# humansensinglab/AGenDA

Measured on AMD Instinct MI355X. Metric: 512x512 images/sec + DAAM heatmaps, 50 DDIM steps, SD-1.5, higher is better.
Workload: dtype bf16

## Files before the change

agenda_amd/csrc/attention.hip:

```cpp
#include "kernels.h"
#include <type_traits>

#ifdef AGD_EXPERIMENTS
int g_attn_qb = 1;
extern "C" __attribute__((visibility("default"))) void agd_set_attn_qb(int v) { g_attn_qb = v; }
#else
constexpr int g_attn_qb = 1;
#endif

template <int D> struct AttnCfg {
  static constexpr int KSTEPS = (D + 15) / 16;
  static constexpr int DBLK = (D + 31) / 32;
  static constexpr int KCH = KSTEPS * 2;
  static constexpr int KPITCH = ((KCH | 1)) * 16;
  static constexpr int VPITCH = ((DBLK | 1)) * 64;
  static constexpr int CH = D / 8;
  static constexpr bool ONES = (DBLK * 32 > D);
  static constexpr bool QPAD = (KSTEPS * 16 > D);
};

#define DEFER_THR 8.0f

template <int D, int KB, int QB, int RECORD, int AMASK = 0, int EXTRA = 0>
#if defined(AGD_EXPERIMENTS) && defined(EXP_ATTN_LB)
#define ATTN_LB(def) ((!RECORD && !AMASK) ? EXP_ATTN_LB : (def))
#else
#define ATTN_LB(def) (def)
#endif
__global__ __launch_bounds__(256, ATTN_LB((AMASK ? 1 : (QB == 1 && D <= 64 && !RECORD) ? 3 : (QB == 1 && D <= 80) ? 2 : 1))) void attn_kernel(const AttnP p) {
  using C = AttnCfg<D>;
  constexpr int KEYS = KB * 32;
  constexpr int KSTEPS = C::KSTEPS, DBLK = C::DBLK, KPITCH = C::KPITCH, VPITCH = C::VPITCH, CH = C::CH;
  constexpr bool ONES = C::ONES && !RECORD;
  constexpr bool QPAD = C::QPAD && !RECORD;
  constexpr bool CNEG = !QPAD && !RECORD;
  constexpr int NCHUNK = KEYS * CH;
  constexpr int LD_IT = (NCHUNK + 255) / 256;
  constexpr int STAGE = KEYS * (KPITCH + VPITCH);
  constexpr int NSTAGE = (RECORD == 1) ? 1 : 2;
  extern __shared__ __attribute__((aligned(16))) char smem[];

  const int tid = threadIdx.x, lane = tid & 63, wid = tid >> 6;
  const int c = lane & 31, hh = lane >> 5;
  const int HPB = (RECORD == 2) ? p.H / p.rec_hpb : p.H;
  const int nqt = p.nqt, nbh = p.B * HPB;
  int bh, qt;
  {
    const int id = blockIdx.x, x = id & 7, j = id >> 3;
    const int per = (nbh + 7) >> 3;
    const int lb = j / nqt;
    qt = j - lb * nqt;
    bh = x * per + lb;
  }
  if (bh >= nbh) return;
  const int hgrp = bh % HPB;
  int head = (RECORD == 2) ? hgrp * p.rec_hpb : hgrp;
  const int hend = (RECORD == 2) ? head + p.rec_hpb : head + 1;
  const int b = bh / HPB;
  const int q0 = qt * (128 * QB) + wid * (32 * QB);
  const bf16_t* kp = p.k + b * p.sk + head * D;
  const bf16_t* vp = p.v + b * p.sv + head * D;

// ... 115 lines not shown
#pragma unroll
      for (int j = 0; j < 16; ++j) oacc[qb][i][j] = 0.f;
  float m_run[QB], l_run[QB];
  f32x16 negm[CNEG ? QB : 1];
#pragma unroll
  for (int qb = 0; qb < QB; ++qb) {
    m_run[qb] = RECORD ? -INFINITY : 0.f; l_run[qb] = 0.f;
    if constexpr (CNEG) {
#pragma unroll
      for (int j = 0; j < 16; ++j) negm[qb][j] = 0.f;
    }
  }
  const float sc = qscale;
  f32x16 pacc[RECORD == 2 ? KB : 1];
  const bool recb = RECORD == 2 && p.record_mode == 3 && b >= p.rec_b0;
  if constexpr (RECORD == 2) {
#pragma unroll
    for (int kb = 0; kb < KB; ++kb)
#pragma unroll
      for (int j = 0; j < 16; ++j) pacc[kb][j] = 0.f;
  }

  const int ntiles_main = RECORD ? 1 : (p.Nk + KEYS - 1) / KEYS;
  const int ntiles = ntiles_main + (EXTRA ? 1 : 0);
  const bool ragged = (p.Nk % KEYS) != 0 || p.causal || AMASK;
  gload(0);
  lstore(0);
  __syncthreads();

  const int gi = lane & 15;
  const int tr_row = (gi >> 2) + 4 * hh;
  const int tr_col = ((lane >> 4) & 1) * 16 + (gi & 3) * 4;

  auto tile_body = [&](int t, auto mask_tag) {
    constexpr bool MASK = decltype(mask_tag)::value;
    const int cur = (RECORD == 1) ? 0 : (RECORD == 2) ? ((t - (hend - p.rec_hpb)) & 1) : (t & 1);
    const char* sK = smem + cur * STAGE;
    const char* sV = sK + KEYS * KPITCH;
    if constexpr (RECORD == 2) { if (t + 1 < hend) { gload_head(t + 1); prefetch_q(t + 1); } }
    else if constexpr (EXTRA) { if (t + 1 < ntiles_main) gload(t + 1); else if (t + 1 == ntiles_main) gload_extra(); }
    else if (t + 1 < ntiles) gload(t + 1);
    f32x16 sacc[QB][KB];
#pragma unroll
    for (int kb = 0; kb < KB; ++kb) {
#pragma unroll
      for (int s = 0; s < KSTEPS; ++s) {
        const bf16x8 a = *(const bf16x8*)(sK + (kb * 32 + c) * KPITCH + (2 * s + hh) * 16);
#pragma unroll
        for (int qb = 0; qb < QB; ++qb) {
          if (s == 0) { const f32x16 z = {0.f, 0.f, 0.f, 0.f, 0.f, 0.f, 0.f, 0.f, 0.f, 0.f, 0.f, 0.f, 0.f, 0.f, 0.f, 0.f};
                        sacc[qb][kb] = __builtin_amdgcn_mfma_f32_32x32x16_bf16(a, qf[qb][s], CNEG ? negm[qb] : z, 0, 0, 0); }
          else sacc[qb][kb] = __builtin_amdgcn_mfma_f32_32x32x16_bf16(a, qf[qb][s], sacc[qb][kb], 0, 0, 0);
        }
      }
    }
    if constexpr (MASK) {
#pragma unroll
      for (int qb = 0; qb < QB; ++qb)
#pragma unroll
        for (int kb = 0; kb < KB; ++kb)
#pragma unroll
          for (int i = 0; i < 16; ++i) {
            const int key = (RECORD || (EXTRA && t == ntiles_main) ? 0 : t * KEYS) + kb * 32 + (i & 3) + 8 * (i >> 2) + 4 * hh;
            if (key >= ((EXTRA && t == ntiles_main) ? p.Nk2 : p.Nk) || (p.causal && key > q0 + qb * 32 + c)) sacc[qb][kb][i] = -INFINITY;
            else if constexpr (AMASK) {
              const float a = p.mask[(long long)b * p.Nk + key];
              sacc[qb][kb][i] += RECORD ? a / p.scale : a * 1.44269504088896340736f;
            }
          }
    }
#pragma unroll
    for (int qb = 0; qb < QB; ++qb) {
      float mx = sacc[qb][0][0];
#pragma unroll
      for (int kb = 0; kb < KB; ++kb)
#pragma unroll
        for (int i = 0; i < 16; ++i) mx = fmaxf(mx, sacc[qb][kb][i]);
      if constexpr (RECORD) {
        mx = xhalf_max(mx) * sc;
        m_run[qb] = mx;
        if constexpr (RECORD == 2) l_run[qb] = 0.f;
        const float nm = -mx;
        float rs = 0.f;
#pragma unroll
        for (int kb = 0; kb < KB; ++kb)
#pragma unroll
          for (int i = 0; i < 16; ++i) {
            const float pv = __builtin_amdgcn_exp2f(fmaf(sacc[qb][kb][i], sc, nm));
            sacc[qb][kb][i] = pv;
            rs += pv;
          }
        l_run[qb] += rs;
      } else {
        if (t == 0 || !__all(mx <= DEFER_THR)) {
          const float mxf = xhalf_max(mx);
          float delta = (t == 0) ? mxf : fmaxf(mxf, 0.f);
          if (!(delta > -INFINITY)) delta = 0.f;
          if constexpr (QPAD) {
            const float mb = (float)(__bf16)(m_run[qb] + delta);
            delta = mb - m_run[qb];
            constexpr int pc = D - 16 * (KSTEPS - 1);
            if (hh == pc / 8) qf[qb][KSTEPS - 1][pc % 8] = (__bf16)(-mb);
          }
          const float alpha = __builtin_amdgcn_exp2f(-delta);
          m_run[qb] += delta;
          l_run[qb] *= alpha;
#pragma unroll
          for (int db = 0; db < DBLK; ++db)
#pragma unroll
            for (int j = 0; j < 16; ++j) oacc[qb][db][j] *= alpha;
#pragma unroll
          for (int kb = 0; kb < KB; ++kb)
#pragma unroll
            for (int i = 0; i < 16; ++i) sacc[qb][kb][i] -= delta;
          if constexpr (CNEG) {
            const float nm = -m_run[qb];
#pragma unroll
            for (int j = 0; j < 16; ++j) negm[qb][j] = nm;
          }
        }
        if constexpr (CNEG) asm volatile("" : "+v"(negm[qb]));
        if constexpr (ONES) {
#pragma unroll
          for (int kb = 0; kb < KB; ++kb)
#pragma unroll
            for (int i = 0; i < 16; ++i) sacc[qb][kb][i] = __builtin_amdgcn_exp2f(sacc[qb][kb][i]);
        } else {
// ... 44 lines not shown
              __builtin_amdgcn_raw_buffer_store_b32(__builtin_bit_cast(unsigned, old[i] + sacc[0][kb][i] * inv), rsrc, off, 0, 0);
            }
          }
        }
      }
    }

#pragma unroll
    for (int kb = 0; kb < KB; ++kb)
#pragma unroll
      for (int s = 0; s < 2; ++s) {
        bf16x8 pf[QB];
#pragma unroll
        for (int qb = 0; qb < QB; ++qb)
#pragma unroll
          for (int j = 0; j < 8; ++j) pf[qb][j] = (__bf16)sacc[qb][kb][8 * s + j];
        const char* vb = sV + (kb * 32 + 16 * s + tr_row) * VPITCH + tr_col * 2;
#pragma unroll
        for (int db = 0; db < DBLK; ++db) {
          const s16x4 lo = __builtin_amdgcn_ds_read_tr16_b64_v4i16((__attribute__((address_space(3))) s16x4*)(vb + db * 64));
          const s16x4 hi = __builtin_amdgcn_ds_read_tr16_b64_v4i16((__attribute__((address_space(3))) s16x4*)(vb + 8 * VPITCH + db * 64));
          const u32x2 lo2 = __builtin_bit_cast(u32x2, lo), hi2 = __builtin_bit_cast(u32x2, hi);
          const u32x4 a4 = u32x4{lo2[0], lo2[1], hi2[0], hi2[1]};
#pragma unroll
          for (int qb = 0; qb < QB; ++qb)
            oacc[qb][db] = __builtin_amdgcn_mfma_f32_32x32x16_bf16(__builtin_bit_cast(bf16x8, a4), pf[qb], oacc[qb][db], 0, 0, 0);
        }
      }
    if ((RECORD == 2) ? (t + 1 < hend) : (t + 1 < ntiles)) {
      lstore(cur ^ 1);
      __syncthreads();
    }
  };
  auto store_o = [&]() {
#pragma unroll
    for (int qb = 0; qb < QB; ++qb) {
      float lt;
      if constexpr (ONES) {
        constexpr int ld = D % 32;
        const float lv = oacc[qb][D / 32][4 * (ld / 8)];
        lt = __shfl(lv, c);
      } else {
        lt = xhalf_sum(l_run[qb]);
      }
      const float inv = 1.0f / lt;
      const int qrow = q0 + qb * 32 + c;
      if (qrow < p.Nq) {
        bf16_t* op = p.o + b * p.so + (long long)qrow * p.ldo + head * D;
#pragma unroll
        for (int db = 0; db < DBLK; ++db)
#pragma unroll
          for (int g = 0; g < 4; ++g) {
            const int d0 = db * 32 + 8 * g + 4 * hh;
            if (d0 < D) {
              u32x2 pk;
              pk[0] = pack_bf2(oacc[qb][db][4 * g + 0] * inv, oacc[qb][db][4 * g + 1] * inv);
              pk[1] = pack_bf2(oacc[qb][db][4 * g + 2] * inv, oacc[qb][db][4 * g + 3] * inv);
              *(u32x2*)(op + d0) = pk;
            }
          }
      }
    }
  };
  {
    using T_ = std::integral_constant<bool, true>; using F_ = std::integral_constant<bool, false>;
    if constexpr (RECORD == 2) {
      const int h0 = head;
      for (; head < hend; ++head) {
        if (head > h0) {
#pragma unroll
          for (int s = 0; s < KSTEPS; ++s) qf[0][s] = __builtin_bit_cast(bf16x8, qnext[s]);
#pragma unroll
          for (int db = 0; db < DBLK; ++db)
#pragma unroll
            for (int j = 0; j < 16; ++j) oacc[0][db][j] = 0.f;
        }
        tile_body(head, T_{});
        store_o();
      }
      if (recb && (q0 + c) < p.Nq) {
        float* base = p.rec + (long long)(b - p.rec_b0) * p.rec_img_stride + hgrp * p.rec_head_stride;
        const unsigned nbytes = (unsigned)p.rec_T * (unsigned)p.Nq * 4u;
        const auto rsrc = __builtin_amdgcn_make_buffer_rsrc(base, 0, nbytes, 0x00020000);
        const unsigned rowb = (unsigned)p.Nq * 4u;
        const unsigned voff0 = (unsigned)(q0 + c) * 4u + (unsigned)(4 * hh) * rowb;
        float old[KB][16];
#pragma unroll
        for (int kb = 0; kb < KB; ++kb)
#pragma unroll
          for (int i = 0; i < 16; ++i)
            old[kb][i] = __builtin_bit_cast(float, __builtin_amdgcn_raw_buffer_load_b32(rsrc, voff0 + (unsigned)(kb * 32 + (i & 3) + 8 * (i >> 2)) * rowb, 0, 0));
#pragma unroll
        for (int kb = 0; kb < KB; ++kb)
#pragma unroll
          for (int i = 0; i < 16; ++i)
            __builtin_amdgcn_raw_buffer_store_b32(__builtin_bit_cast(unsigned, old[kb][i] + pacc[kb][i]), rsrc,
                                                  voff0 + (unsigned)(kb * 32 + (i & 3) + 8 * (i >> 2)) * rowb, 0, 0);
      }
      return;
    } else if constexpr (RECORD) {
      tile_body(0, T_{});
    } else if constexpr (EXTRA) {
      for (int t = 0; t < ntiles_main - 1; ++t) tile_body(t, F_{});
      if (ragged) tile_body(ntiles_main - 1, T_{}); else tile_body(ntiles_main - 1, F_{});
      tile_body(ntiles_main, T_{});
    } else {
      if (p.causal || AMASK) { for (int t = 0; t < ntiles - 1; ++t) tile_body(t, T_{}); }
      else { for (int t = 0; t < ntiles - 1; ++t) tile_body(t, F_{}); }
      if (ragged) tile_body(ntiles - 1, T_{}); else tile_body(ntiles - 1, F_{});
    }
  }
  store_o();
}


template <int D, int KB, int QB, int RECORD, int AMASK = 0, int EXTRA = 0>
static int launch_attn_t(const AttnP& p, hipStream_t st) {
  using C = AttnCfg<D>;
  constexpr int lds = (RECORD == 1 ? 1 : 2) * KB * 32 * (C::KPITCH + C::VPITCH);
  AttnP pp = p;
  pp.nqt = (p.Nq + 128 * QB - 1) / (128 * QB);
  const int per = (p.B * (RECORD == 2 ? p.H / p.rec_hpb : p.H) + 7) / 8;
  dim3 grid(8 * per * pp.nqt);
  auto kfn = attn_kernel<D, KB, QB, RECORD, AMASK, EXTRA>;
  if (lds > 65536) {
    static std::atomic<bool> attr[AGD_MAX_DEVICES] = {};
    int dev = 0; HIP_CHECK_RET(hipGetDevice(&dev));
    if (dev < 0 || dev >= AGD_MAX_DEVICES) { agd_set_error("attention: device ordinal %d out of range", dev); return -1; }
    if (!attr[dev]) { HIP_CHECK_RET(hipFuncSetAttribute((const void*)kfn, hipFuncAttributeMaxDynamicSharedMemorySize, lds)); attr[dev] = true; }
  }
  hipLaunchKernelGGL(kfn, grid, dim3(256), lds, st, pp);
  HIP_CHECK_RET(hipGetLastError());
  return 0;
}

template <int D>
static int launch_attn_d(const AttnP& p, hipStream_t st) {
  if (p.k2) {
    if (p.record_mode != 0 || p.mask || p.causal) { agd_set_error("attention: a second K/V source takes no recording, mask or causal order"); return -1; }
    if (!p.v2 || p.Nk2 < 1 || p.Nk2 > 64 || ((p.ldk2 | p.ldv2) & 7)) { agd_set_error("attention: second K/V source of %d keys (1 .. 64, pitches multiples of 8)", p.Nk2); return -1; }
    return launch_attn_t<D, 2, 1, 0, 0, 1>(p, st);
  }
  if (p.record_mode != 0) {
    if (p.Nk > 96) { agd_set_error("attention: recording needs Nk <= 96 (got %d)", p.Nk); return -1; }
    if (p.record_mode == 3) {
      if (p.mask) { agd_set_error("attention: head-summed recording does not take an attention mask"); return -1; }
      if (p.rec_hpb < 1 || p.H % p.rec_hpb) { agd_set_error("attention: rec_hpb %d does not divide %d heads", p.rec_hpb, p.H); return -1; }
      return launch_attn_t<D, 3, 1, 2>(p, st);
    }
    return p.mask ? launch_attn_t<D, 3, 1, 1, 1>(p, st) : launch_attn_t<D, 3, 1, 1>(p, st);
  }
  if (p.mask) {
    if (p.causal) { agd_set_error("attention: additive mask + causal unsupported"); return -1; }
    return (p.Nk <= 96 && p.Nk > 64) ? launch_attn_t<D, 3, 1, 0, 1>(p, st) : launch_attn_t<D, 2, 1, 0, 1>(p, st);
  }
  if (p.Nk <= 96 && p.Nk > 64) return launch_attn_t<D, 3, 1, 0>(p, st);
  if constexpr (D <= 80) { if (p.Nq >= 1024 && g_attn_qb == 2) return launch_attn_t<D, 2, 2, 0>(p, st); }
#if defined(AGD_EXPERIMENTS) && defined(EXP_ATTN_KB)
  if (p.Nk >= 1024) return launch_attn_t<D, EXP_ATTN_KB, 1, 0>(p, st);
#endif
  return launch_attn_t<D, 2, 1, 0>(p, st);
}

int launch_attention(const AttnP& p, hipStream_t st) {
  if ((p.ldq | p.ldk | p.ldv | p.ldo) & 3) { agd_set_error("attention: row pitches must be multiples of 4 elements"); return -1; }
  if ((p.ldq | p.ldk | p.ldv) & 7) { agd_set_error("attention: q/k/v pitches must be multiples of 8 elements"); return -1; }
  switch (p.D) {
    case 32: return launch_attn_d<32>(p, st);
    case 40: return launch_attn_d<40>(p, st);
    case 64: return launch_attn_d<64>(p, st);
    case 80: return launch_attn_d<80>(p, st);
    case 128: return launch_attn_d<128>(p, st);
    case 160: return launch_attn_d<160>(p, st);
    default: agd_set_error("attention: unsupported head dim %d", p.D); return -1;
  }
}
```

agenda_amd/csrc/kernels.h:

```cpp
#pragma once
#include "common.h"

#define AGD_MAX_DEVICES 16
struct SplitKWs { float* p = nullptr; size_t cap = 0; };

struct IgemmP {
  const bf16_t* sc0 = nullptr; const bf16_t* sc1 = nullptr; int sc_C0 = 0, sc_C1 = 0;
  int ups4 = 0;
  const bf16_t* src0; const bf16_t* src1;
  int C0, C1;
  int Hin, Win, Hout, Wout;
  int ksize, stride, pad, up;
  const bf16_t* W;
  const float* bias; int bias_mode;
  const float* rowadd; int rowadd_ld;
  const bf16_t* residual; int ldr;
  void* out; int out_f32; int ldo;
  int M, N, K;
  float alpha;
  int geglu;
  int act;
  int batch;
  long long sA0, sA1, sW, sO, sR;
  const bf16_t* zero_page;
// ... 6 lines not shown
  int* cfg_out;
  int w_per_image;
  int wmajor;
  int warm;
  int halo;
  int p8;
  const float* gn_gamma; const float* gn_beta; bf16_t* gn_y; int gn_groups; float gn_eps; int gn_silu; int gn_keep_out; int* gn_fused;
  int kg2;
  int smap;
  int wreg, wreg_mmin, wreg_mmax;
  const bf16_t* Wfrag; int wfrag_ni;
  int xb_m, xb_n;
  int xcd_block;
  int pc;
  int stagger;
  int dbg;
};
int launch_igemm(const IgemmP& p, hipStream_t st);
int igemm_query(const IgemmP& p, int* cfg3);

struct AttnP {
  const bf16_t* q; const bf16_t* k; const bf16_t* v; bf16_t* o;
  int ldq, ldk, ldv, ldo;
  long long sq, sk, sv, so;
  int B, H, D, Nq, Nk;
  float scale;
  int record_mode; int rec_b0;
  float* rec; long long rec_img_stride; long long rec_head_stride;
  int rec_T;
  int rec_hpb;
  int nqt;
  int causal;
  const float* mask;
  const bf16_t* k2; const bf16_t* v2; int ldk2, ldv2; long long sk2, sv2; int Nk2;
};
int launch_attention(const AttnP& p, hipStream_t st);

struct FFusedP {
  const bf16_t* h; bf16_t* out;
  const bf16_t* w1f;
  const float* cs1; const float* b1;
  const bf16_t* w2f;
  const float* b2;
  int M; float ln_eps;
  const bf16_t* wpf; const float* bp; const bf16_t* xres; bf16_t* pout; float* colstat;
  int xres_rows;
  int premul;
};
int launch_ff_fused(const FFusedP& p, int C, hipStream_t st);
struct AttnChainP {
  const bf16_t* h; bf16_t* out;
  const float* gamma; const float* beta; float ln_eps;
  const bf16_t* wqf;
  const bf16_t* wof; const float* bo;
  const bf16_t* kv; int ldkv; long long skv;
  int M, HW, T; float scale;
  int record; float* rec; long long rec_img_stride, rec_head_stride; int rec_T, rec_b0, rec_hpb;
  float* rowstat_out;
  const bf16_t* o1; const bf16_t* wo1f; const float* bo1;
  int rows32;
  int src_rows;
};
int launch_attn_chain(const AttnChainP& p, int C, int heads, hipStream_t st);
struct QkvChainP {
  const bf16_t* x;
  const bf16_t* wbf; long long wb_stride; const float* rowadd;
// ... 154 lines not shown
```

agenda_amd/csrc/model.hip:

```cpp
#include "../../include/agenda_hip.h"
#include "kernels.h"

#include <algorithm>
#include <cmath>
#include <cstdarg>
#include <cstdio>
#include <cstring>
#include <functional>
#include <string>
#include <unordered_map>
#include <vector>

static thread_local char g_err[2048] = "";
#define AGD_API extern "C" __attribute__((visibility("default")))
extern "C" void agd_set_error(const char* fmt, ...) {
  va_list ap; va_start(ap, fmt); vsnprintf(g_err, sizeof(g_err), fmt, ap); va_end(ap);
}
#define CK(expr) do { if ((expr) != 0) return -1; } while (0)
#define FAIL(...) do { agd_set_error(__VA_ARGS__); return -1; } while (0)

struct WMat { bf16_t* w = nullptr; int N = 0, Cin = 0, Cpad = 0, taps = 0;
              int sc_cols = 0;
              bf16_t* wfrag = nullptr; int wfrag_ni = 0; };
struct Act { bf16_t* p = nullptr; int B = 0, H = 0, W = 0, C = 0; float* cpart = nullptr; int cpart_bm = 0;
// ... 38 lines not shown
  int acc_heads = 0;
  DBuf wqTb, wkvTb, woTb; WMat wqT, wkvT, woT;
  bf16_t* pm_wqT = nullptr; float* pm_wqb = nullptr; bool pm_ready = false;
  DBuf pm_kppb, pm_vppb, pm_csb; bf16_t* pm_kpp = nullptr; bf16_t* pm_vpp = nullptr; float* pm_kcs = nullptr; float* pm_kbs = nullptr;
};

struct Fuser {
  std::string pre; int C = 0, heads = 0;
  WMat wqkv, wkv; float ta = 0.f, td = 0.f; float* bo_s = nullptr; float* b2_s = nullptr;
  DBuf gkvb;
};

struct IpaLayer {
  std::string pre; int C = 0, heads = 0, cols = 0;
  DBuf wk, wv, kppb, vppb, csbsb;
};

enum : int {
  TBF_FF            = 1 << 0,
  TBF_ATTN2         = 1 << 1,
  TBF_ATTN1_OUT     = 1 << 2,
  TBF_FF_PROJ       = 1 << 3,
  TBF_QKV           = 1 << 4,
  TBF_ATTN2_640     = 1 << 5,
  TBF_LAZY_DUP      = 1 << 6,
  TBF_QKV_GN        = 1 << 7,
  TBF_QKV_640       = 1 << 8,
  TBF_FF_PREMUL     = 1 << 9,
  TBF_ATTN2_ROWS32  = 1 << 10,
  TBF_QKV_ROWS64    = 1 << 11,
  TBF_QKV_SCHED2    = 1 << 12,
  TBF_DEFAULT       = 0x1fff & ~TBF_QKV_640,
};

struct ProfEv { int cls; double flops, bytes; hipEvent_t a, b; };

struct EvalCond {
  float cn_scale = 0.f;
  bool grounded = false;
  float ad_scale = 0.f;
  bool ipa = false;
};

struct agd_ctx {
  int device = 0; agd_config cfg{}; std::string err;
  std::unordered_map<std::string, WMat> W;
  std::unordered_map<std::string, float*> V;
  std::unordered_map<std::string, int> Vn;
  std::vector<void*> owned;
  Arena arena; bf16_t* zero_page = nullptr;
  float* stage = nullptr; size_t stage_bytes = 0;
  bool finalized = false;
  WMat tproj_all; float* tproj_bias = nullptr; float* tproj_out = nullptr; int tproj_total = 0;
  const float* tproj_cur = nullptr;
  int tproj_cur_ld = 0;
  float* tsteps_buf = nullptr; int tsteps_cap = 0;
  std::unordered_map<std::string, int> tproj_off;
  float* temb_buf = nullptr;
  float* t_dev = nullptr;
  std::vector<XLayer> xl; std::unordered_map<std::string, int> xl_idx;
  DBuf ctxb; bf16_t* ctx_bf16 = nullptr; int ctx_B2 = 0, ctx_T = 0;
  int rec_mode = 0, rec_is_train = 0, rec_T_cfg = 0, rec_T = 0, rec_B = 0, rec_L = 0, rec_Lh = 0, rec_Lw = 0;
  DBuf hook_sumb, hook_scratchb, hook_headsb, hook_storeb;
  struct HookRec { size_t off; int Bp, T, N; };
  std::vector<HookRec> hook_recs; size_t hook_store_used = 0;
  DBuf bwd_wsb;
  float* hook_sum = nullptr; float* hook_scratch = nullptr; int hook_count = 0, hook_Bp = 0, hook_T = 0;
  int rec_base = 0, rec_call = 0;
  int pano_B = 0, pano_Lh = 0, pano_Lw = 0, pano_stride = 0;
  DBuf pano_ctxb;
  DBuf pano_viewb, pano_hmb;
  DBuf latb, epsb, vae_imgb, plmsb, dpmb;
  bf16_t* lat_bf16 = nullptr; float* eps_nhwc = nullptr;
  SplitKWs splitk;
  int opt_cfg_share = 1;
  int opt_ln_fold = 1;
  int opt_gn_fused = 1;
  int opt_warm = 3;
  int opt_gn_proj_fold = 1;
  int opt_p8 = 1;
  int opt_halo = 1;
  int opt_tb_fuse = TBF_DEFAULT;
  int opt_ups4 = 7;
  int opt_ffproj = 1;
  int opt_sc_fuse = 3;
  int opt_wreg = 3;
  int opt_kg2 = 1;
  int opt_side = 0;
  hipStream_t side = nullptr; hipEvent_t ev_fork = nullptr, ev_join = nullptr;
  int opt_smap = 1;
  int opt_reduce_gn = 1;
  int opt_xcd_block = 1;
  int opt_pc = 49;
  agd_vision_config vis{}; bool vis_on = false; float* vis_concepts = nullptr;
  agd_vision_config ienc{}; int ienc_state = 0;
  int opt_xpre = 1;
  int opt_touch = 3;
  unsigned* touch_sink = nullptr;
  agd_controlnet_config cnc{}; bool cn_on = false;
  WMat cn_tproj_all; float* cn_tproj_bias = nullptr; float* cn_tproj_out = nullptr; int cn_tproj_total = 0;
  int cn_nres = 0; float* cn_zb = nullptr; float* cn_zbs = nullptr; int cn_zb_total = 0; std::vector<int> cn_zb_off; float cn_zscale = NAN;
  DBuf cn_embb; int cn_emb_B2 = 0, cn_emb_Lh = 0, cn_emb_Lw = 0, cn_emb_rep = 0;
  std::vector<float> cn_sched;
  int ip_mode = 0, ip_B = 0, ip_Lh = 0, ip_Lw = 0, ip_Cm = 0, ip_Cc = 0;
  DBuf ip_maskb, ip_condb, ip_noiseb;
  std::vector<float> ip_sched;
  bool i2_on = false; int i2_B = 0, i2_Lh = 0, i2_Lw = 0; float i2_scale = 1.f;
  int i2_prep_B = 0, i2_prep_Lh = 0, i2_prep_Lw = 0;
  DBuf i2_latb;
  std::vector<std::string> lora_keys; std::vector<LoraMergeD> lora_d; int lora_tiles = 0;
  DBuf lora_descb; bf16_t* lora_scratch = nullptr; size_t lora_scratch_n = 0;
  float lora_scale = 0.f; bool lora_dirty = false;
// ... 253 lines not shown
    c->arena.release(mk);
    return 0;
  }
  if (side_out) {
    if (hipStreamWaitEvent(st, c->ev_join, 0) != hipSuccess) FAIL("side stream wait");
    res = side_out;
  } else if (has_sc) {
    GETW(ws, pre + "conv_shortcut.weight"); GETV(bs, pre + "conv_shortcut.bias");
    GemmOpt os; os.bias = bs;
    CK(run_conv(c, st, x0.p, x0.C, x1 ? x1->p : nullptr, C1, B, H, Wd, *ws, 1, h.p, os, c->zero_page));
    res = h.p;
  } else if (x1 || x0.C != Cout) {
    FAIL("resnet %s: channel change %d->%d without conv_shortcut", pre.c_str(), Cin, Cout);
  }
  GETW(w2, pre + "conv2.weight"); GETV(cb2, pre + "conv2.bias");
  GemmOpt o2; o2.bias = cb2; o2.residual = res; o2.out_act = &out;
  int gn2_done = 0;
  if (out_normed) {
    o2.gn_gamma = next->gamma; o2.gn_beta = next->beta; o2.gn_y = out_normed; o2.gn_groups = groups; o2.gn_eps = next->eps; o2.gn_silu = next->silu;
    o2.gn_keep_out = 1; o2.gn_fused = &gn2_done;
  }
  CK(run_conv(c, st, n2.p, Cout, nullptr, 0, B, H, Wd, *w2, 3, out.p, o2, c->zero_page));
  if (gn2_done) { out.normed = out_normed; out.normed_gamma = next->gamma; }
  c->arena.release(mk);
  return 0;
}

static int run_attention(agd_ctx* c, hipStream_t st, int cls, AttnP& a) {
  const double fl = 4.0 * a.B * a.H * (double)a.Nq * a.Nk * a.D;
  double by = 2.0 * a.B * a.H * (double)a.D * (2.0 * a.Nq + 2.0 * a.Nk);
  if (a.record_mode == 1) by += 8.0 * (a.B - a.rec_b0) * a.H * (double)a.rec_T * a.Nq;
  else if (a.record_mode == 2 || a.record_mode == 3) by += 8.0 * (a.B - a.rec_b0) * (double)a.rec_T * a.Nq;
  ProfScope ps(c, st, cls, fl, by);
  return launch_attention(a, st);
}

static inline bool daam_records(const agd_ctx* c, const XLayer& xl, int B2, int qh, int qw) {
  return c->rec_mode == 1 && !xl.mid && xl.acc && c->rec_Lh / qh != 8 && qh == xl.acc_h && qw == xl.acc_w && B2 / 2 == rec_images(c);
}

static int cross_attention(agd_ctx* c, hipStream_t st, XLayer& xl, const bf16_t* q, int B2, int N, int qh, int qw, bf16_t* out, bool record,
                           const float* mask = nullptr) {
  const int C = xl.C, D = C / xl.heads, T = c->ctx_T;
  if (xl.cn) record = false;
  AttnP a{}; a.q = q; a.k = xl.kv; a.v = xl.kv + C; a.o = out;
  a.ldq = C; a.ldk = 2 * C; a.ldv = 2 * C; a.ldo = C;
  a.sq = (long long)N * C; a.sk = (long long)T * 2 * C; a.sv = a.sk; a.so = a.sq;
  a.B = B2; a.H = xl.heads; a.D = D; a.Nq = N; a.Nk = T; a.scale = 1.0f / sqrtf((float)D);
  a.record_mode = 0; a.mask = mask;
  const int side = qh;
  bool hook_call = false;
  if (record && daam_records(c, xl, B2, qh, qw)) {
    a.rec_b0 = B2 / 2; a.rec_T = c->rec_T;
    a.rec_head_stride = (long long)c->rec_T * N; a.rec_img_stride = a.rec_head_stride * xl.acc_heads;
    a.rec = xl.acc + (size_t)c->rec_base * a.rec_img_stride;
    if (xl.acc_heads < xl.heads) {
      if (mask) FAIL("attention_mask together with daam recording at latent resolution is not supported");
      a.record_mode = 3; a.rec_hpb = xl.heads / xl.acc_heads;
    } else a.record_mode = 1;
  } else if (record && c->rec_mode == 2 && c->hook_scratch) {
    const int b0 = c->rec_is_train ? 0 : B2 / 2;
    if (B2 - b0 == c->hook_Bp) {
      if (qh != qw) FAIL("the hook.py recorder takes square maps only (h = w = sqrt(N)); this call's map is %d x %d", qh, qw);
      if (T != c->hook_T || side > c->rec_L) FAIL("hook recorder was reset for %d tokens / latent side %d but this call has %d tokens / side %d: call clear() (agd_record_reset) after changing the context", c->hook_T, c->rec_L, T, side);
      const size_t nh = (size_t)c->hook_Bp * xl.heads * T * N;
      CK(c->hook_headsb.ensure(nh * 4));
// ... 1819 lines not shown
    const float* f; CK(guidance_factor(c, st, eps, batch, Cl, HW, guidance, &f));
    return launch_cfg_dpm(eps, c->cfg.out_channels, latents, prev, store, batch, Cl, HW, guidance, coeffs + (size_t)5 * i, f, st);
  }));
  return 0;
}
AGD_API int agd_denoise_dpm(agd_ctx* c, float* latents, int batch, int L, int n_evals, const float* timesteps, const float* coeffs,
                            float guidance, void* stream) {
  return agd_denoise_dpm_hw(c, latents, batch, L, L, n_evals, timesteps, coeffs, guidance, stream);
}

AGD_API int agd_vae_decode_hw(agd_ctx* c, const float* latents, int batch, int Lh, int Lw, unsigned char* out_u8, float* out_f32, void* stream) {
  API_CK(c, need_final(c));
  if (Lh < 1 || Lw < 1) { agd_set_error("vae_decode: latent size %d x %d", Lh, Lw); return fail_ctx(c); }
  hipStream_t st = S(stream);
  API_CK(c, ensure_lat(c, batch, Lh, Lw));
  const int sh = c->cfg.vae_n_levels - 1;
  const long long npix = (long long)batch * (Lh << sh) * (Lw << sh);
  { ProfScope ps(c, st, PC_ELEM, 0);
    API_CK(c, launch_prep_latents(latents, c->lat_bf16, batch, c->cfg.vae_latent_channels, Lh * Lw, 64, 1, 1.0f / c->cfg.vae_scaling_factor, st)); }
  API_CK(c, c->vae_imgb.ensure((size_t)npix * 4 * 4));
  float* img = c->vae_imgb.as<float>();
  int rc = vae_walk(c, st, c->lat_bf16, batch, Lh, Lw, img);
  if (rc == 0 && out_u8) { ProfScope ps(c, st, PC_ELEM, 0); rc = launch_image_u8(img, 4, out_u8, npix, c->cfg.vae_out_channels, st); }
  if (rc == 0 && out_f32) {
    rc = launch_nchw_from_nhwc_f32(img, 4, out_f32, (int)npix, c->cfg.vae_out_channels, 1, st);
  }
  return rc ? fail_ctx(c) : 0;
}
AGD_API int agd_vae_decode(agd_ctx* c, const float* latents, int batch, int L, unsigned char* out_u8, float* out_f32, void* stream) {
  return agd_vae_decode_hw(c, latents, batch, L, L, out_u8, out_f32, stream);
}

AGD_API int agd_set_option(agd_ctx* c, const char* name, int value) {
  if (!c || !name) { agd_set_error("set_option: null argument"); return fail_ctx(c); }
  if (!strcmp(name, "cfg_shared_prefix")) { c->opt_cfg_share = value != 0; return 0; }
  if (!strcmp(name, "ln_fold")) { c->opt_ln_fold = value; return 0; }
  if (!strcmp(name, "gn_fused_stats")) { c->opt_gn_fused = value != 0; return 0; }
  if (!strcmp(name, "weight_touch")) { c->opt_touch = value < 0 ? 0 : value; return 0; }
  if (!strcmp(name, "weight_warm")) { c->opt_warm = value; return 0; }
  if (!strcmp(name, "conv_halo")) { c->opt_halo = value != 0; return 0; }
  if (!strcmp(name, "gn_proj_fold")) { c->opt_gn_proj_fold = value < 0 ? 0 : value; return 0; }
  if (!strcmp(name, "tblock_fuse")) { c->opt_tb_fuse = value < 0 ? 0 : value; return 0; }
  if (!strcmp(name, "reduce_gn")) { c->opt_reduce_gn = value != 0; return 0; }
  if (!strcmp(name, "xcd_block")) { c->opt_xcd_block = value != 0; return 0; }
  if (!strcmp(name, "igemm_pc")) { c->opt_pc = value < 0 ? 0 : value; return 0; }
  if (!strcmp(name, "attn2_premul")) { c->opt_xpre = value < 0 ? 0 : value; return 0; }
  if (!strcmp(name, "conv_smap")) { c->opt_smap = value != 0; return 0; }
  if (!strcmp(name, "side_stream")) { c->opt_side = value < 0 ? 0 : value; return 0; }
  if (!strcmp(name, "igemm_kgroups")) { c->opt_kg2 = value != 0; return 0; }
  if (!strcmp(name, "upsample_phases")) { c->opt_ups4 = value & 15; return 0; }
  if (!strcmp(name, "ff_proj_fuse")) { c->opt_ffproj = value != 0; return 0; }
  if (!strcmp(name, "shortcut_fuse")) { c->opt_sc_fuse = value & 3; return 0; }
  if (!strcmp(name, "wreg_mask")) { c->opt_wreg = value & 3; return 0; }
  if (!strcmp(name, "igemm8p")) { c->opt_p8 = value < 0 ? 0 : value; return 0; }
  agd_set_error("set_option: unknown option '%s'", name);
  return fail_ctx(c);
}

AGD_API int agd_record_config(agd_ctx* c, int mode, int is_train, int rec_tokens) {
  if (!c) return -1;
  if (mode < 0 || mode > 2) { agd_set_error("record_config: mode %d", mode); return fail_ctx(c); }
  c->rec_mode = mode; c->rec_is_train = is_train; c->rec_T_cfg = rec_tokens;
  return 0;
}

static int hook_reset_rows(agd_ctx* c, int rows, int L, hipStream_t st) {
  const int Tc = c->ctx_T > 0 ? c->ctx_T : c->cfg.max_tokens;
// ... 471 lines not shown
  CK(launch_convert_weight(wo, wob, C, C, 1, C, 0, st));
  CK(launch_matvec_bf16(wqb, beta, wqbeta, C, C, st));
  CK(launch_rowstat_bf16(xb, rst, (int)M, C, st));
  XattnPremulP pm{}; pm.kv = kvb; pm.ldkv = 2 * C; pm.skv = (long long)T * 2 * C; pm.wqT = wqT; pm.wo = wob; pm.gamma = gamma; pm.wqb = wqbeta;
  pm.B = B; pm.T = T; pm.C = C; pm.H = heads; pm.scale = 1.0f / sqrtf((float)(C / heads)); pm.kpp = kpp; pm.kcs = kcs; pm.kbs = kcs + (size_t)B * HT; pm.vpp = vpp;
  CK(launch_xattn_premul(pm, st));
  XattnSP sp{}; sp.x = xb; sp.ln_stats = rst; sp.ln_slots = 1; sp.ln_invC = 1.0f / (float)C; sp.ln_eps = eps; sp.kpp = kpp; sp.kcs = pm.kcs; sp.kbs = pm.kbs; sp.P = P;
  sp.M = (int)M; sp.HW = HW; sp.C = C; sp.H = heads; sp.T = T;
  if (probs) {
    if (hipMemsetAsync(probs, 0, (size_t)B * heads * T * HW * 4, st) != hipSuccess) { agd_set_error("memset probs"); return -1; }
    sp.rec = probs; sp.rec_b0 = 0; sp.rec_T = T; sp.rec_head_stride = (long long)T * HW; sp.rec_img_stride = sp.rec_head_stride * heads;
  }
  CK(launch_xattn_s(sp, st));
  WMat wv; wv.w = vpp; wv.N = C; wv.Cin = (int)HT; wv.Cpad = (int)HT; wv.taps = 1;
  GemmOpt oo; oo.bias = bo; oo.residual = xb; oo.w_per_image = 1;
  CK(run_conv(nullptr, st, P, (int)HT, nullptr, 0, B, 1, HW, wv, 1, yb, oo, op_zero_page()));
  CK(launch_bf16_to_f32(yb, y, M * C, st));
  hipStreamSynchronize(st);
  return 0;
}

AGD_API int agd_op_attention(const float* q, const float* k, const float* v, float* o, int B, int H, int D, int Nq, int Nk,
                                float scale, float* probs_out, void* stream) {
  hipStream_t st = S(stream); Tmp tmp;
  const int C = H * D;
  bf16_t* qb = tmp.get<bf16_t>((size_t)B * Nq * C); bf16_t* kb = tmp.get<bf16_t>((size_t)B * Nk * C);
  bf16_t* vb = tmp.get<bf16_t>((size_t)B * Nk * C); bf16_t* ob = tmp.get<bf16_t>((size_t)B * Nq * C);
  if (!qb || !kb || !vb || !ob) return -1;
  CK(launch_f32_to_bf16(q, qb, (long long)B * Nq * C, st));
  CK(launch_f32_to_bf16(k, kb, (long long)B * Nk * C, st));
  CK(launch_f32_to_bf16(v, vb, (long long)B * Nk * C, st));
  AttnP a{}; a.q = qb; a.k = kb; a.v = vb; a.o = ob; a.ldq = a.ldk = a.ldv = a.ldo = C;
  a.sq = (long long)Nq * C; a.so = a.sq; a.sk = (long long)Nk * C; a.sv = a.sk;
  a.B = B; a.H = H; a.D = D; a.Nq = Nq; a.Nk = Nk; a.scale = scale;
  if (probs_out) {
    if (hipMemsetAsync(probs_out, 0, (size_t)B * H * Nk * Nq * 4, st) != hipSuccess) { agd_set_error("memset probs"); return -1; }
    a.record_mode = 1; a.rec_b0 = 0; a.rec = probs_out; a.rec_T = Nk;
    a.rec_head_stride = (long long)Nk * Nq; a.rec_img_stride = a.rec_head_stride * H;
  }
  CK(launch_attention(a, st));
  CK(launch_bf16_to_f32(ob, o, (long long)B * Nq * C, st));
  hipStreamSynchronize(st);
  return 0;
}

AGD_API int agd_op_attention_headsum(const float* q, const float* k, const float* v, float* o, int B, int H, int D, int Nq, int Nk,
                                     float scale, float* probs_sum_out, void* stream) {
  hipStream_t st = S(stream); Tmp tmp;
  const int C = H * D;
  if (!probs_sum_out) { agd_set_error("attention_headsum: probs_sum_out is required"); return -1; }
  bf16_t* qb = tmp.get<bf16_t>((size_t)B * Nq * C); bf16_t* kb = tmp.get<bf16_t>((size_t)B * Nk * C);
  bf16_t* vb = tmp.get<bf16_t>((size_t)B * Nk * C); bf16_t* ob = tmp.get<bf16_t>((size_t)B * Nq * C);
  if (!qb || !kb || !vb || !ob) return -1;
  CK(launch_f32_to_bf16(q, qb, (long long)B * Nq * C, st));
  CK(launch_f32_to_bf16(k, kb, (long long)B * Nk * C, st));
  CK(launch_f32_to_bf16(v, vb, (long long)B * Nk * C, st));
  AttnP a{}; a.q = qb; a.k = kb; a.v = vb; a.o = ob; a.ldq = a.ldk = a.ldv = a.ldo = C;
  a.sq = (long long)Nq * C; a.so = a.sq; a.sk = (long long)Nk * C; a.sv = a.sk;
  a.B = B; a.H = H; a.D = D; a.Nq = Nq; a.Nk = Nk; a.scale = scale;
  if (hipMemsetAsync(probs_sum_out, 0, (size_t)B * Nk * Nq * 4, st) != hipSuccess) { agd_set_error("memset probs"); return -1; }
  a.record_mode = 3; a.rec_hpb = H; a.rec_b0 = 0; a.rec = probs_sum_out; a.rec_T = Nk; a.rec_img_stride = (long long)Nk * Nq;
  CK(launch_attention(a, st));
  CK(launch_bf16_to_f32(ob, o, (long long)B * Nq * C, st));
  hipStreamSynchronize(st);
  return 0;
}

// ... 200 lines not shown
    if (!qkv || !part || !gv) return -1;
    hipMemset(part, 0x3C, (size_t)B * (HW / 128) * C * 2 * 4); hipMemset(gv, 0x3C, (size_t)4 * C * 4);
    CK(launch_frag_order_w(w2, w2f, C, C, 5, C, 0)); CK(launch_frag_order_w(w1, w1f, 3 * C, C, 5, C, 0));
    qp.x = h; qp.wbf = w2f; qp.wb_stride = 0; qp.rowadd = gv; qp.rowadd_stride = 0; qp.h = o; qp.gamma = gv + C; qp.beta = gv + 2 * C; qp.ln_eps = 1e-5f;
    qp.wqkvf = w1f; qp.qkv = qkv; qp.M = (int)M; qp.HW = HW; qp.rows64 = kind == 7 || kind == 9; qp.sched2 = kind >= 8;
    qp.gn_part = part; qp.gn_bm = 128; qp.gn_groups = 32; qp.gn_eps = 1e-6f; qp.gn_gamma = gv + 3 * C; qp.gn_beta = gv;
  }
  auto run = [&]() { return qkvk ? launch_qkv_chain(qp, C, 0) : (kind == 0 || kind == 2) ? launch_ff_fused(fp, C, 0) : launch_attn_chain(ap, C, 8, 0); };
  hipEvent_t a, b; hipEventCreate(&a); hipEventCreate(&b);
  for (int i = 0; i < 2; ++i) CK(run());
  hipEventRecord(a, 0);
  for (int i = 0; i < iters; ++i) CK(run());
  hipEventRecord(b, 0); hipEventSynchronize(b);
  float t = 0; hipEventElapsedTime(&t, a, b);
  *ms_out = t / iters;
  hipEventDestroy(a); hipEventDestroy(b);
  return 0;
}

AGD_API int agd_bench_attention(int B, int H, int D, int Nq, int Nk, int record, int iters, double* ms_out) {
  Tmp tmp;
  const int C = H * D;
  const bool self = (Nq == Nk);
  bf16_t* q = tmp.get<bf16_t>((size_t)B * Nq * (self ? 3 * C : C)); bf16_t* kv = self ? nullptr : tmp.get<bf16_t>((size_t)B * Nk * 2 * C);
  bf16_t* o = tmp.get<bf16_t>((size_t)B * Nq * C);
  float* rec = record ? tmp.get<float>((size_t)B * H * Nk * Nq) : nullptr;
  if (!q || !o || (!self && !kv) || (record && !rec)) return -1;
  fill_rand(q, (long long)B * Nq * (self ? 3 * C : C), 5, 1.0f); if (kv) fill_rand(kv, (long long)B * Nk * 2 * C, 6, 1.0f);
  if (rec) hipMemset(rec, 0, (size_t)B * H * Nk * Nq * 4);
  AttnP a{};
  if (self) { a.q = q; a.k = q + C; a.v = q + 2 * C; a.ldq = a.ldk = a.ldv = 3 * C; a.sq = a.sk = a.sv = (long long)Nq * 3 * C; }
  else { a.q = q; a.k = kv; a.v = kv + C; a.ldq = C; a.ldk = a.ldv = 2 * C; a.sq = (long long)Nq * C; a.sk = a.sv = (long long)Nk * 2 * C; }
  a.o = o; a.ldo = C; a.so = (long long)Nq * C; a.B = B; a.H = H; a.D = D; a.Nq = Nq; a.Nk = Nk; a.scale = 1.0f / sqrtf((float)D);
  if (record) { a.record_mode = record >= 2 ? 3 : 1; a.rec_hpb = record >= 2 ? (16 >> record < H ? 16 >> record : H) : 0; a.rec_b0 = B / 2; a.rec = rec;
                a.rec_T = Nk; a.rec_head_stride = (long long)Nk * Nq; a.rec_img_stride = a.rec_head_stride * (record >= 2 ? H / a.rec_hpb : H); }
  hipEvent_t e0, e1; hipEventCreate(&e0); hipEventCreate(&e1);
  for (int i = 0; i < 2; ++i) CK(launch_attention(a, 0));
  hipEventRecord(e0, 0);
  for (int i = 0; i < iters; ++i) CK(launch_attention(a, 0));
  hipEventRecord(e1, 0); hipEventSynchronize(e1);
  float t = 0; hipEventElapsedTime(&t, e0, e1);
  *ms_out = t / iters;
  hipEventDestroy(e0); hipEventDestroy(e1);
  return 0;
}

AGD_API int agd_bench_groupnorm_ex(int B, int HW, int C0, int C1, int fused_stats, int iters, double* ms_out) {
  Tmp tmp;
  const int C = C0 + C1;
  if (B < 1 || HW < 1 || C0 < 8 || C1 < 0 || iters < 1 || !ms_out) { agd_set_error("bench_groupnorm: bad arguments"); return -1; }
  bf16_t* x0 = tmp.get<bf16_t>((size_t)B * HW * C0); bf16_t* x1 = C1 ? tmp.get<bf16_t>((size_t)B * HW * C1) : nullptr;
  bf16_t* y = tmp.get<bf16_t>((size_t)B * HW * C);
  float* ws = tmp.get<float>((size_t)groupnorm_ws_floats(B, C, HW, 32)); float* g = tmp.get<float>(2 * C);
  if (!x0 || (C1 && !x1) || !y || !ws || !g) return -1;
  fill_rand(x0, (long long)B * HW * C0, 7, 1.0f); if (C1) fill_rand(x1, (long long)B * HW * C1, 8, 1.0f);
  hipMemset(g, 0, 2 * C * 4);
  GroupNormP p{}; p.x0 = x0; p.x1 = x1; p.C0 = C0; p.C1 = C1; p.y = y; p.gamma = g; p.beta = g + C; p.B = B; p.HW = HW; p.groups = 32; p.eps = 1e-5f; p.silu = 1; p.ws = ws;
  if (fused_stats) {
    if (HW % 128) { agd_set_error("bench_groupnorm: fused_stats needs HW %% 128 == 0"); return -1; }
    const size_t n0 = (size_t)B * (HW / 128) * C0 * 2, n1 = (size_t)B * (HW / 128) * C1 * 2;
    float* p0 = tmp.get<float>(n0); float* p1 = C1 ? tmp.get<float>(n1) : nullptr;
    if (!p0 || (C1 && !p1)) return -1;
    hipMemset(p0, 0, n0 * 4); if (C1) hipMemset(p1, 0, n1 * 4);
    p.part0 = p0; p.part1 = p1; p.bm0 = 128; p.bm1 = C1 ? 128 : 0;
  }
  hipEvent_t e0, e1; hipEventCreate(&e0); hipEventCreate(&e1);
// ... 1114 lines not shown
```

agenda_amd/ops.py:

```python
from __future__ import annotations

import torch

from . import _lib


def _f32c(t):
    assert t.is_cuda, "ops run on the GPU only (no CPU fallback)"
    return t.detach().to(torch.float32).contiguous()


_P8 = {0: 0, 1: 2, 2: 4, 3: 8}


def conv2d(x, w, bias=None, stride=1, padding=None, upsample=False, halo=False, p8=0, smap=False, phases=False, pc=0, xcd_block=False):
    lib = _lib.load()
    x, w = _f32c(x), _f32c(w)
    b = _f32c(bias) if bias is not None else None
    B, Cin, H, W = x.shape
    Cout, _, k, _ = w.shape
    pad = (1 if k == 3 else 0) if padding is None else padding
    up = 2 if upsample else 1
    Ho = (H * up + 2 * pad - k) // stride + 1
    Wo = (W * up + 2 * pad - k) // stride + 1
# ... 45 lines not shown
    Cc = x.shape[-1]
    x2 = _f32c(x).reshape(-1, Cc)
    y = torch.empty_like(x2)
    _lib.check(lib.agd_op_ff_fused(_lib.ptr(x2), _lib.ptr(_f32c(gamma)), _lib.ptr(_f32c(beta)), _lib.ptr(_f32c(w1)), _lib.ptr(_f32c(b1)),
                                   _lib.ptr(_f32c(w2)), _lib.ptr(_f32c(b2)), _lib.ptr(y), x2.shape[0], Cc, float(eps),
                                   _lib.current_stream_ptr()), None, "agd_op_ff_fused")
    return y.reshape(x.shape)


def attn_chain(x, gamma, beta, wq, kv, wo, bo, heads=8, eps=1e-5, return_probs=False, rows32=False):
    lib = _lib.load()
    x, kv = _f32c(x), _f32c(kv)
    B, HW, Cc = x.shape
    T = kv.shape[1]
    y = torch.empty_like(x)
    pr = torch.empty(B, T, HW, device=x.device, dtype=torch.float32) if return_probs else None
    _lib.check(lib.agd_op_attn_chain(_lib.ptr(x), _lib.ptr(_f32c(gamma)), _lib.ptr(_f32c(beta)), _lib.ptr(_f32c(wq)), _lib.ptr(kv), _lib.ptr(_f32c(wo)),
                                     _lib.ptr(_f32c(bo)), _lib.ptr(y), _lib.ptr(pr), B, HW, T, Cc, heads | (256 if rows32 else 0), float(eps), _lib.current_stream_ptr()),
               None, "agd_op_attn_chain")
    return (y, pr) if return_probs else y


def xattn_premul(x, gamma, beta, wq, kv, wo, bo, heads=8, eps=1e-5, return_probs=False):
    lib = _lib.load()
    x, kv = _f32c(x), _f32c(kv)
    B, HW, Cc = x.shape
    T = kv.shape[1]
    y = torch.empty_like(x)
    pr = torch.empty(B, heads, T, HW, device=x.device, dtype=torch.float32) if return_probs else None
    _lib.check(lib.agd_op_xattn_premul(_lib.ptr(x), _lib.ptr(_f32c(gamma)), _lib.ptr(_f32c(beta)), _lib.ptr(_f32c(wq)), _lib.ptr(kv), _lib.ptr(_f32c(wo)),
                                       _lib.ptr(_f32c(bo)), _lib.ptr(y), _lib.ptr(pr), B, HW, T, Cc, heads, float(eps), _lib.current_stream_ptr()),
               None, "agd_op_xattn_premul")
    return (y, pr) if return_probs else y


def attention(q, k, v, heads, scale=None, return_probs=False):
    lib = _lib.load()
    q, k, v = _f32c(q), _f32c(k), _f32c(v)
    B, Nq, Cc = q.shape
    Nk = k.shape[1]
    D = Cc // heads
    scale = D ** -0.5 if scale is None else scale
    o = torch.empty_like(q)
    probs = torch.empty(B, heads, Nk, Nq, device=q.device, dtype=torch.float32) if return_probs else None
    _lib.check(lib.agd_op_attention(_lib.ptr(q), _lib.ptr(k), _lib.ptr(v), _lib.ptr(o), B, heads, D, Nq, Nk, float(scale),
                                    _lib.ptr(probs), _lib.current_stream_ptr()), None, "agd_op_attention")
    return (o, probs) if return_probs else o


def attention_headsum(q, k, v, heads, scale=None):
    lib = _lib.load()
    q, k, v = _f32c(q), _f32c(k), _f32c(v)
    B, Nq, Cc = q.shape
    Nk = k.shape[1]
    D = Cc // heads
    scale = D ** -0.5 if scale is None else scale
    o = torch.empty_like(q)
    probs = torch.empty(B, Nk, Nq, device=q.device, dtype=torch.float32)
    _lib.check(lib.agd_op_attention_headsum(_lib.ptr(q), _lib.ptr(k), _lib.ptr(v), _lib.ptr(o), B, heads, D, Nq, Nk, float(scale),
                                            _lib.ptr(probs), _lib.current_stream_ptr()), None, "agd_op_attention_headsum")
    return o, probs


def attention_backward(q, kv, heads, d_o=None, d_map=None, b0=0, scale=None):
    lib = _lib.load()
    q, kv = _f32c(q), _f32c(kv)
# ... 123 lines not shown
```

Baseline: 8.897.

## Use fixed softmax reference in flash attention with overflow fallback recompute

Adds a FIXREF variant of the plain flash-attention kernel that skips the per-tile row-max computation and rescaling after the first tile, using the first tile's max as a fixed reference. After all tiles it checks for overflow or non-finite results across the block and, only if any are found, resets the accumulators and reruns the normal online-softmax path. This removes per-tile max reductions, cross-lane shuffles and oacc rescales, at the cost of a block-wide vote and a possible full recompute on blocks that overflow. It is enabled by default for non-causal attention.

Result: no change. 8.924, median of 6 (+0.3%).

```diff
diff --git a/agenda_amd/csrc/attention.hip b/agenda_amd/csrc/attention.hip
--- a/agenda_amd/csrc/attention.hip
+++ b/agenda_amd/csrc/attention.hip
@@ -21,13 +21,14 @@
 
 #define DEFER_THR 8.0f
 
-template <int D, int KB, int QB, int RECORD, int AMASK = 0, int EXTRA = 0>
+template <int D, int KB, int QB, int RECORD, int AMASK = 0, int EXTRA = 0, int FIXREF = 0>
 #if defined(AGD_EXPERIMENTS) && defined(EXP_ATTN_LB)
 #define ATTN_LB(def) ((!RECORD && !AMASK) ? EXP_ATTN_LB : (def))
 #else
 #define ATTN_LB(def) (def)
 #endif
 __global__ __launch_bounds__(256, ATTN_LB((AMASK ? 1 : (QB == 1 && D <= 64 && !RECORD) ? 3 : (QB == 1 && D <= 80) ? 2 : 1))) void attn_kernel(const AttnP p) {
+  static_assert(!FIXREF || (!RECORD && !AMASK && !EXTRA), "FIXREF: the plain flash instantiations only");
   using C = AttnCfg<D>;
   constexpr int KEYS = KB * 32;
   constexpr int KSTEPS = C::KSTEPS, DBLK = C::DBLK, KPITCH = C::KPITCH, VPITCH = C::VPITCH, CH = C::CH;
@@ -209,14 +210,16 @@
   const int tr_row = (gi >> 2) + 4 * hh;
   const int tr_col = ((lane >> 4) & 1) * 16 + (gi & 3) * 4;
 
-  auto tile_body = [&](int t, auto mask_tag) {
+  auto tile_body = [&](int t, auto mask_tag, auto fix_tag) {
     constexpr bool MASK = decltype(mask_tag)::value;
+    constexpr bool FIX = decltype(fix_tag)::value;
     const int cur = (RECORD == 1) ? 0 : (RECORD == 2) ? ((t - (hend - p.rec_hpb)) & 1) : (t & 1);
     const char* sK = smem + cur * STAGE;
     const char* sV = sK + KEYS * KPITCH;
     if constexpr (RECORD == 2) { if (t + 1 < hend) { gload_head(t + 1); prefetch_q(t + 1); } }
     else if constexpr (EXTRA) { if (t + 1 < ntiles_main) gload(t + 1); else if (t + 1 == ntiles_main) gload_extra(); }
     else if (t + 1 < ntiles) gload(t + 1);
+    if constexpr (FIX) __builtin_amdgcn_sched_barrier(0);
     f32x16 sacc[QB][KB];
 #pragma unroll
     for (int kb = 0; kb < KB; ++kb) {
@@ -248,11 +251,14 @@
     }
 #pragma unroll
     for (int qb = 0; qb < QB; ++qb) {
-      float mx = sacc[qb][0][0];
-#pragma unroll
-      for (int kb = 0; kb < KB; ++kb)
-#pragma unroll
-        for (int i = 0; i < 16; ++i) mx = fmaxf(mx, sacc[qb][kb][i]);
+      float mx = 0.f;
+      if constexpr (!FIX) {
+        mx = sacc[qb][0][0];
+#pragma unroll
+        for (int kb = 0; kb < KB; ++kb)
+#pragma unroll
+          for (int i = 0; i < 16; ++i) mx = fmaxf(mx, sacc[qb][kb][i]);
+      }
       if constexpr (RECORD) {
         mx = xhalf_max(mx) * sc;
         m_run[qb] = mx;
@@ -269,7 +275,7 @@
           }
         l_run[qb] += rs;
       } else {
-        if (t == 0 || !__all(mx <= DEFER_THR)) {
+        if constexpr (!FIX) if (t == 0 || !__all(mx <= DEFER_THR)) {
           const float mxf = xhalf_max(mx);
           float delta = (t == 0) ? mxf : fmaxf(mxf, 0.f);
           if (!(delta > -INFINITY)) delta = 0.f;
@@ -380,17 +386,19 @@
       __syncthreads();
     }
   };
+  auto row_sum = [&](int qb) {
+    if constexpr (ONES) {
+      constexpr int ld = D % 32;
+      const float lv = oacc[qb][D / 32][4 * (ld / 8)];
+      return __shfl(lv, c);
+    } else {
+      return xhalf_sum(l_run[qb]);
+    }
+  };
   auto store_o = [&]() {
 #pragma unroll
     for (int qb = 0; qb < QB; ++qb) {
-      float lt;
-      if constexpr (ONES) {
-        constexpr int ld = D % 32;
-        const float lv = oacc[qb][D / 32][4 * (ld / 8)];
-        lt = __shfl(lv, c);
-      } else {
-        lt = xhalf_sum(l_run[qb]);
-      }
+      const float lt = row_sum(qb);
       const float inv = 1.0f / lt;
       const int qrow = q0 + qb * 32 + c;
       if (qrow < p.Nq) {
@@ -423,7 +431,7 @@
 #pragma unroll
             for (int j = 0; j < 16; ++j) oacc[0][db][j] = 0.f;
         }
-        tile_body(head, T_{});
+        tile_body(head, T_{}, F_{});
         store_o();
       }
       if (recb && (q0 + c) < p.Nq) {
@@ -447,22 +455,59 @@
       }
       return;
     } else if constexpr (RECORD) {
-      tile_body(0, T_{});
+      tile_body(0, T_{}, F_{});
     } else if constexpr (EXTRA) {
-      for (int t = 0; t < ntiles_main - 1; ++t) tile_body(t, F_{});
-      if (ragged) tile_body(ntiles_main - 1, T_{}); else tile_body(ntiles_main - 1, F_{});
-      tile_body(ntiles_main, T_{});
+      for (int t = 0; t < ntiles_main - 1; ++t) tile_body(t, F_{}, F_{});
+      if (ragged) tile_body(ntiles_main - 1, T_{}, F_{}); else tile_body(ntiles_main - 1, F_{}, F_{});
+      tile_body(ntiles_main, T_{}, F_{});
     } else {
-      if (p.causal || AMASK) { for (int t = 0; t < ntiles - 1; ++t) tile_body(t, T_{}); }
-      else { for (int t = 0; t < ntiles - 1; ++t) tile_body(t, F_{}); }
-      if (ragged) tile_body(ntiles - 1, T_{}); else tile_body(ntiles - 1, F_{});
+      if constexpr (FIXREF) {
+        if (ntiles == 1) { if (ragged) tile_body(0, T_{}, F_{}); else tile_body(0, F_{}, F_{}); }
+        else {
+          tile_body(0, F_{}, F_{});
+          for (int t = 1; t < ntiles - 1; ++t) tile_body(t, F_{}, T_{});
+          if (ragged) tile_body(ntiles - 1, T_{}, T_{}); else tile_body(ntiles - 1, F_{}, T_{});
+        }
+        bool bad = false;
+#pragma unroll
+        for (int qb = 0; qb < QB; ++qb) {
+          bad |= !(row_sum(qb) < 0x1p100f);
+#pragma unroll
+          for (int db = 0; db < DBLK; ++db)
+#pragma unroll
+            for (int j = 0; j < 16; ++j) bad |= !(fabsf(oacc[qb][db][j]) < INFINITY);
+        }
+        if (!__syncthreads_or(bad)) { store_o(); return; }
+#pragma unroll
+        for (int qb = 0; qb < QB; ++qb) {
+#pragma unroll
+          for (int db = 0; db < DBLK; ++db)
+#pragma unroll
+            for (int j = 0; j < 16; ++j) oacc[qb][db][j] = 0.f;
+          m_run[qb] = 0.f; l_run[qb] = 0.f;
+          if constexpr (QPAD) {
+            constexpr int pc = D - 16 * (KSTEPS - 1);
+            if (hh == pc / 8) qf[qb][KSTEPS - 1][pc % 8] = (__bf16)0.f;
+          }
+          if constexpr (CNEG) {
+#pragma unroll
+            for (int j = 0; j < 16; ++j) negm[qb][j] = 0.f;
+          }
+        }
+        gload(0);
+        lstore(0);
+        __syncthreads();
+      }
+      if (p.causal || AMASK) { for (int t = 0; t < ntiles - 1; ++t) tile_body(t, T_{}, F_{}); }
+      else { for (int t = 0; t < ntiles - 1; ++t) tile_body(t, F_{}, F_{}); }
+      if (ragged) tile_body(ntiles - 1, T_{}, F_{}); else tile_body(ntiles - 1, F_{}, F_{});
     }
   }
   store_o();
 }
 
 
-template <int D, int KB, int QB, int RECORD, int AMASK = 0, int EXTRA = 0>
+template <int D, int KB, int QB, int RECORD, int AMASK = 0, int EXTRA = 0, int FIXREF = 0>
 static int launch_attn_t(const AttnP& p, hipStream_t st) {
   using C = AttnCfg<D>;
   constexpr int lds = (RECORD == 1 ? 1 : 2) * KB * 32 * (C::KPITCH + C::VPITCH);
@@ -470,7 +515,7 @@
   pp.nqt = (p.Nq + 128 * QB - 1) / (128 * QB);
   const int per = (p.B * (RECORD == 2 ? p.H / p.rec_hpb : p.H) + 7) / 8;
   dim3 grid(8 * per * pp.nqt);
-  auto kfn = attn_kernel<D, KB, QB, RECORD, AMASK, EXTRA>;
+  auto kfn = attn_kernel<D, KB, QB, RECORD, AMASK, EXTRA, FIXREF>;
   if (lds > 65536) {
     static std::atomic<bool> attr[AGD_MAX_DEVICES] = {};
     int dev = 0; HIP_CHECK_RET(hipGetDevice(&dev));
@@ -507,6 +552,7 @@
 #if defined(AGD_EXPERIMENTS) && defined(EXP_ATTN_KB)
   if (p.Nk >= 1024) return launch_attn_t<D, EXP_ATTN_KB, 1, 0>(p, st);
 #endif
+  if (p.fixed_ref && !p.causal) return launch_attn_t<D, 2, 1, 0, 0, 0, 1>(p, st);
   return launch_attn_t<D, 2, 1, 0>(p, st);
 }
 
diff --git a/agenda_amd/csrc/kernels.h b/agenda_amd/csrc/kernels.h
--- a/agenda_amd/csrc/kernels.h
+++ b/agenda_amd/csrc/kernels.h
@@ -62,6 +62,7 @@
   int nqt;
   int causal;
   const float* mask;
+  int fixed_ref;
   const bf16_t* k2; const bf16_t* v2; int ldk2, ldv2; long long sk2, sv2; int Nk2;
 };
 int launch_attention(const AttnP& p, hipStream_t st);
diff --git a/agenda_amd/csrc/model.hip b/agenda_amd/csrc/model.hip
--- a/agenda_amd/csrc/model.hip
+++ b/agenda_amd/csrc/model.hip
@@ -94,6 +94,8 @@
   TBF_QKV_SCHED2    = 1 << 12,
   TBF_DEFAULT       = 0x1fff & ~TBF_QKV_640,
 };
+
+static std::atomic<int> g_attn_fixed_ref{1};
 
 struct ProfEv { int cls; double flops, bytes; hipEvent_t a, b; };
 
@@ -140,6 +142,7 @@
   int opt_gn_fused = 1;
   int opt_warm = 3;
   int opt_gn_proj_fold = 1;
+  int opt_attn_fixref = g_attn_fixed_ref;
   int opt_p8 = 1;
   int opt_halo = 1;
   int opt_tb_fuse = TBF_DEFAULT;
@@ -459,6 +462,7 @@
   if (a.record_mode == 1) by += 8.0 * (a.B - a.rec_b0) * a.H * (double)a.rec_T * a.Nq;
   else if (a.record_mode == 2 || a.record_mode == 3) by += 8.0 * (a.B - a.rec_b0) * (double)a.rec_T * a.Nq;
   ProfScope ps(c, st, cls, fl, by);
+  a.fixed_ref = c->opt_attn_fixref;
   return launch_attention(a, st);
 }
 
@@ -2344,7 +2348,9 @@
 }
 
 AGD_API int agd_set_option(agd_ctx* c, const char* name, int value) {
+  if (!c && name && !strcmp(name, "attn_fixed_ref")) { g_attn_fixed_ref = value != 0; return 0; }
   if (!c || !name) { agd_set_error("set_option: null argument"); return fail_ctx(c); }
+  if (!strcmp(name, "attn_fixed_ref")) { c->opt_attn_fixref = value != 0; return 0; }
   if (!strcmp(name, "cfg_shared_prefix")) { c->opt_cfg_share = value != 0; return 0; }
   if (!strcmp(name, "ln_fold")) { c->opt_ln_fold = value; return 0; }
   if (!strcmp(name, "gn_fused_stats")) { c->opt_gn_fused = value != 0; return 0; }
@@ -2882,7 +2888,7 @@
   CK(launch_f32_to_bf16(v, vb, (long long)B * Nk * C, st));
   AttnP a{}; a.q = qb; a.k = kb; a.v = vb; a.o = ob; a.ldq = a.ldk = a.ldv = a.ldo = C;
   a.sq = (long long)Nq * C; a.so = a.sq; a.sk = (long long)Nk * C; a.sv = a.sk;
-  a.B = B; a.H = H; a.D = D; a.Nq = Nq; a.Nk = Nk; a.scale = scale;
+  a.B = B; a.H = H; a.D = D; a.Nq = Nq; a.Nk = Nk; a.scale = scale; a.fixed_ref = g_attn_fixed_ref;
   if (probs_out) {
     if (hipMemsetAsync(probs_out, 0, (size_t)B * H * Nk * Nq * 4, st) != hipSuccess) { agd_set_error("memset probs"); return -1; }
     a.record_mode = 1; a.rec_b0 = 0; a.rec = probs_out; a.rec_T = Nk;
@@ -3149,6 +3155,7 @@
   if (self) { a.q = q; a.k = q + C; a.v = q + 2 * C; a.ldq = a.ldk = a.ldv = 3 * C; a.sq = a.sk = a.sv = (long long)Nq * 3 * C; }
   else { a.q = q; a.k = kv; a.v = kv + C; a.ldq = C; a.ldk = a.ldv = 2 * C; a.sq = (long long)Nq * C; a.sk = a.sv = (long long)Nk * 2 * C; }
   a.o = o; a.ldo = C; a.so = (long long)Nq * C; a.B = B; a.H = H; a.D = D; a.Nq = Nq; a.Nk = Nk; a.scale = 1.0f / sqrtf((float)D);
+  a.fixed_ref = g_attn_fixed_ref;
   if (record) { a.record_mode = record >= 2 ? 3 : 1; a.rec_hpb = record >= 2 ? (16 >> record < H ? 16 >> record : H) : 0; a.rec_b0 = B / 2; a.rec = rec;
                 a.rec_T = Nk; a.rec_head_stride = (long long)Nk * Nq; a.rec_img_stride = a.rec_head_stride * (record >= 2 ? H / a.rec_hpb : H); }
   hipEvent_t e0, e1; hipEventCreate(&e0); hipEventCreate(&e1);
diff --git a/agenda_amd/ops.py b/agenda_amd/ops.py
--- a/agenda_amd/ops.py
+++ b/agenda_amd/ops.py
@@ -101,6 +101,10 @@
                                        _lib.ptr(_f32c(bo)), _lib.ptr(y), _lib.ptr(pr), B, HW, T, Cc, heads, float(eps), _lib.current_stream_ptr()),
                None, "agd_op_xattn_premul")
     return (y, pr) if return_probs else y
+
+
+def set_option(name, value):
+    _lib.check(_lib.load().agd_set_option(None, name.encode(), int(value)), None, f"agd_set_option({name})")
 
 
 def attention(q, k, v, heads, scale=None, return_probs=False):
```
